# liupei101/VLSA

Measured on AMD Instinct MI355X. Metric: patches/sec per slide (50k x 512 CONCH bag), higher is better.
Workload: dtype bf16

## Files before the change

### vlsa_amd/csrc/vlfan_batch.hip

```cpp
#include "vlsa_common.h"
#ifndef VLSA_DMA_NT
#define VLSA_DMA_NT "nt"
#endif

namespace vlsa {

typedef __attribute__((address_space(3))) void* lds_void_ptr;
typedef bf16x8 __attribute__((may_alias)) bf16x8_ma;
typedef f32x4 __attribute__((may_alias)) f32x4_ma;
typedef float __attribute__((may_alias)) float_ma;
typedef int __attribute__((may_alias)) int_ma;
typedef int i32x4 __attribute__((ext_vector_type(4)));

struct BagDesc {
    const void* X;
    int64_t N;
    int64_t ldx;
};
struct RowsDesc {
    float* ptr;
    int64_t ld;
};

#ifdef VLSA_TIMING
// ... 492 lines not shown
    }
    constexpr int U = 8;
    float mx = -INFINITY;
    if (p < P)
        for (int g = 0; g < G; ++g) mx = fmaxf(mx, pm[(size_t)g * st.sm]);
    float4 a = make_float4(0.f, 0.f, 0.f, 0.f);
    float lt = 0.f;
    for (int g0 = gs; g0 < G; g0 += 2 * U) {
        float mg[U], lg[U];
        float4 v[U];
#pragma unroll
        for (int u = 0; u < U; ++u) {
            const int g = g0 + 2 * u;
            const bool ok = live && g < G;
            mg[u] = ok ? pm[(size_t)g * st.sm] : -INFINITY;
            lg[u] = ok ? pl[(size_t)g * st.sl] : 0.f;
            v[u] = ok ? *reinterpret_cast<const float4*>(pacc + (size_t)g * st.sa) : make_float4(0.f, 0.f, 0.f, 0.f);
        }
#pragma unroll
        for (int u = 0; u < U; ++u) {
            const float f = (mg[u] == -INFINITY) ? 0.f : fast_exp2(mg[u] - mx);
            lt += lg[u] * f;
            a.x += v[u].x * f; a.y += v[u].y * f; a.z += v[u].z * f; a.w += v[u].w * f;
        }
    }
    if (gs == 1) {
        sacc[p][c4] = a;
        slt[p][c4] = lt;
    }
    __syncthreads();
    if (gs == 0) {
        const float4 o = sacc[p][c4];
        a.x += o.x; a.y += o.y; a.z += o.z; a.w += o.w;
        lt += slt[p][c4];
        if (live) {
            const float inv = 1.f / lt;
            a.x *= inv; a.y *= inv; a.z *= inv; a.w *= inv;
            *reinterpret_cast<float4*>(out + (size_t)bag * st.oo + (size_t)p * D + col) = a;
            if (blockIdx.x == 0 && c4 == 0) {
                m2[(size_t)bag * st.om + p] = mx;
                l[(size_t)bag * st.ol + p] = lt;
            }
        }
    }
    if (pooled == nullptr) return;
    __syncthreads();
    if (gs == 0) sacc[p][c4] = a;
    __syncthreads();
    if (tid < 16 && col < D) {
        float4 r;
        if (pool_mode == VLSA_POOL_MAX) {
            r = sacc[0][tid];
            for (int q = 1; q < P; ++q) {
                const float4 o = sacc[q][tid];
                r.x = fmaxf(r.x, o.x); r.y = fmaxf(r.y, o.y); r.z = fmaxf(r.z, o.z); r.w = fmaxf(r.w, o.w);
            }
        } else if (pool_mode == VLSA_POOL_WEIGHT) {
            r = make_float4(0.f, 0.f, 0.f, 0.f);
            for (int q = 0; q < P; ++q) {
                const float4 o = sacc[q][tid];
                const float wq = spw[q];
                r.x += wq * o.x; r.y += wq * o.y; r.z += wq * o.z; r.w += wq * o.w;
            }
        } else {
            r = make_float4(0.f, 0.f, 0.f, 0.f);
            for (int q = 0; q < P; ++q) {
                const float4 o = sacc[q][tid];
                r.x += o.x; r.y += o.y; r.z += o.z; r.w += o.w;
            }
            const float fp = (float)P;
            r.x /= fp; r.y /= fp; r.z /= fp; r.w /= fp;
        }
        *reinterpret_cast<float4*>(pooled + (size_t)bag * D + col) = r;
    }
}

__global__ __launch_bounds__(256) void k_vlfan_merge_pool_small(const float* __restrict__ pm, const float* __restrict__ pl,
                                                                    const float* __restrict__ pacc, int G, int P, int D,
                                                                    float* __restrict__ m2, float* __restrict__ l,
                                                                    float* __restrict__ out, MergeStrides st, int pool_mode,
                                                                    const float* __restrict__ pool_w, float* __restrict__ pooled) {
    __shared__ float sm_[8][VLSA_MAX_P], sl_[8][VLSA_MAX_P];
    __shared__ float sinv[VLSA_MAX_P], spw[VLSA_MAX_P];
    __builtin_amdgcn_s_setprio(VLSA_TAIL_PRIO);
    const int tid = threadIdx.x, bag = blockIdx.x;
    pm += (size_t)bag * st.bm;
    pl += (size_t)bag * st.bl;
    pacc += (size_t)bag * st.ba;
    if (tid < 8 * VLSA_MAX_P) {
        const int g = tid >> 4, p = tid & 15;
        const bool ok = g < G && p < P;
        sm_[g][p] = ok ? pm[(size_t)g * st.sm + p] : -INFINITY;
        sl_[g][p] = ok ? pl[(size_t)g * st.sl + p] : 0.f;
    }
    if (pool_mode == VLSA_POOL_WEIGHT && tid == 255) {
        float mx = -INFINITY, sum = 0.f;
        for (int q = 0; q < P; ++q) mx = fmaxf(mx, pool_w[q]);
        for (int q = 0; q < P; ++q) { spw[q] = expf(pool_w[q] - mx); sum += spw[q]; }
        for (int q = 0; q < P; ++q) spw[q] /= sum;
    }
    __syncthreads();
    if (tid < VLSA_MAX_P) {
        const int p = tid;
        float mx = -INFINITY;
#pragma unroll
        for (int g = 0; g < 8; ++g) mx = fmaxf(mx, sm_[g][p]);
        float ls = 0.f;
#pragma unroll
        for (int g = 0; g < 8; ++g) {
            const float f = sm_[g][p] == -INFINITY ? 0.f : fast_exp2(sm_[g][p] - mx);
            ls += sl_[g][p] * f;
            sm_[g][p] = f;
        }
        sinv[p] = 1.f / ls;
        if (p < P) {
            m2[(size_t)bag * st.om + p] = mx;
            l[(size_t)bag * st.ol + p] = ls;
        }
    }
    __syncthreads();
    for (int c = tid; c < D; c += 256) {
        float acc[VLSA_MAX_P];
#pragma unroll
        for (int p = 0; p < VLSA_MAX_P; ++p) acc[p] = 0.f;
        for (int g = 0; g < G; ++g) {
            float x[VLSA_MAX_P];
#pragma unroll
            for (int p = 0; p < VLSA_MAX_P; ++p) x[p] = p < P ? pacc[(size_t)g * st.sa + (size_t)p * D + c] : 0.f;
#pragma unroll
            for (int p = 0; p < VLSA_MAX_P; ++p) acc[p] += x[p] * sm_[g][p];
        }
        float r = pool_mode == VLSA_POOL_MAX ? -INFINITY : 0.f;
#pragma unroll
        for (int p = 0; p < VLSA_MAX_P; ++p)
            if (p < P) {
                const float o = acc[p] * sinv[p];
                out[(size_t)bag * st.oo + (size_t)p * D + c] = o;
                if (pool_mode == VLSA_POOL_MAX) r = fmaxf(r, o);
                else if (pool_mode == VLSA_POOL_WEIGHT) r += spw[p] * o;
                else r += o;
            }
        if (pool_mode == VLSA_POOL_MEAN) r /= (float)P;
        if (pooled != nullptr) pooled[(size_t)bag * D + c] = r;
    }
}

__global__ __launch_bounds__(256) void k_attn_normalise_batch(const BagDesc* __restrict__ bags, const RowsDesc* __restrict__ sdesc,
                                                             const RowsDesc* __restrict__ adesc, const float* __restrict__ m2,
                                                             const float* __restrict__ l, int m_stride) {
    const int bag = blockIdx.z, p = blockIdx.y;
    const int64_t n = ((int64_t)blockIdx.x * 256 + threadIdx.x) * 4;
    const int64_t N = bags[bag].N;
    const RowsDesc sd = sdesc[bag], ad = adesc[bag];
    if (n >= N || sd.ptr == nullptr || ad.ptr == nullptr) return;
    const float m = m2[(size_t)bag * m_stride + p], inv = 1.f / l[(size_t)bag * m_stride + p];
    const f32x4 t = *reinterpret_cast<const f32x4*>(sd.ptr + (size_t)p * sd.ld + n);
    f32x4 a;
#pragma unroll
    for (int r = 0; r < 4; ++r) a[r] = fast_exp2(t[r] - m) * inv;
    *reinterpret_cast<f32x4*>(ad.ptr + (size_t)p * ad.ld + n) = a;
}

}

using namespace vlsa;

int vlsa_launch_head_batch(const float* rows, int B, int P, int D, int pool_mode, const float* pool_w, const float* W,
                           const float* b, const float* That, int K, const float* logit_scale, unsigned int* counters,
                           float* pooled, float* v, float* vhat, float* vnorm, float* logits, float* incidence,
                           hipStream_t s);
int vlsa_launch_head_pooled_batch(const float* pooled, int B, int D, const float* W, const float* b, const float* That, int K,
                                  const float* logit_scale, float* v, float* vhat, float* vnorm, float* logits,
                                  float* incidence, hipStream_t s);
int vlsa_launch_head_rows_batch(const float* rows, int B, int P, int D, int pool_mode, const float* pool_w, const float* W,
                                const float* b, const float* That, int K, const float* logit_scale, float* pooled, float* v,
                                float* vhat, float* vnorm, float* logits, float* incidence, hipStream_t s);

static int launch_merge_pool(const float* pm, const float* pl, const float* pacc, int B, int G, int P, int D, float* m2, float* l,
                             float* out, const MergeStrides& st, int pool_mode, const float* pool_w, float* pooled, hipStream_t s) {
    if (G <= 8)
        hipLaunchKernelGGL(k_vlfan_merge_pool_small, dim3(B), dim3(256), 0, s, pm, pl, pacc, G, P, D, m2, l, out, st, pool_mode, pool_w,
                           pooled);
    else
        hipLaunchKernelGGL(k_vlfan_merge_pool_batch, dim3((D + 63) / 64, B), dim3(512), 0, s, pm, pl, pacc, G, P, D, m2, l, out, st,
                           pool_mode, pool_w, pooled);
    return hipGetLastError() == hipSuccess ? VLSA_OK : VLSA_ELAUNCH;
}

#ifdef VLSA_TIMING
extern "C" int vlsa_debug_read_batch_cycles(long long* host_out) {
    return hipMemcpyFromSymbol(host_out, HIP_SYMBOL(vlsa::vlsa_dbg_batch), sizeof(long long) * 64) == hipSuccess ? 0 : -3;
}
#endif

static inline int batch_groups(int B) { return B >= 8 ? 8 : (B >= 4 ? 4 : (B >= 2 ? 2 : 1)); }
static inline int min_groups(int B) {
    int m = 1;
    while (m * bt::kMaxLocal < B) m *= 2;
    return m;
}
static inline int resolve_groups(int B, int groups) {
    int S = groups > 0 ? groups : batch_groups(B);
    int p2 = 1;
    while (p2 * 2 <= S && p2 * 2 <= B && p2 * 2 <= 256) p2 *= 2;
    const int m = min_groups(B);
    return p2 < m ? m : p2;
}
static inline int batch_workgroups(int S, int reserved_cus) {
    int r = reserved_cus < 0 ? 0 : reserved_cus;
    r = (r + S - 1) / S * S;
    if (r > 256 - S) r = 256 - S;
    return 256 - r;
}
extern "C" int vlsa_batch_partials_per_bag(int B) { return 256 / batch_groups(B); }
extern "C" int vlsa_batch_partials_per_bag_ex(int B, int reserved_cus, int groups) {
    const int S = resolve_groups(B, groups);
    return batch_workgroups(S, reserved_cus) / S;
}
extern "C" int vlsa_batch_groups(const int64_t* rows_host, int B, int reserved_cus) {
    if (!rows_host || B < 1) return 1;
    int best = 1;
    double best_cost = 1e300;
    for (int S = min_groups(B); S <= 256 && S <= B; S *= 2) {
        const int Gb = batch_workgroups(S, reserved_cus) / S;
        double worst = 0.0;
        for (int g = 0; g < S; ++g) {
            double c = 0.0;
            for (int t = g; t < B; t += S) {
                const int64_t units = (rows_host[t] + 63) / 64;
                c += (double)((units + Gb - 1) / Gb) + 0.7;
            }
            if (c > worst) worst = c;
        }
        if (worst < best_cost * 0.999) {
            best_cost = worst;
            best = S;
        }
    }
    return best;
}

extern "C" int vlsa_batch_max_bags(void) { return 64; }
extern "C" int vlsa_batch_forward_max_bags(void) { return bt::kMaxBags; }

extern "C" size_t vlsa_batch_workspace_bytes(int B, int P, int D) {
    const size_t recs = (size_t)(B < bt::kMaxLocal ? B : bt::kMaxLocal) * 256;
    return (recs * kPStride * 2 + recs * P * D) * sizeof(float) + (size_t)B * 64;
}

int vlsa_launch_partial_f32_batch(const void* bag_desc, int B, const float* qeff, const float* qmeta, int P, float* pm,
                                  float* pl, float* pacc, int S, int workgroups, const void* scores_desc, hipStream_t s);

extern "C" int vlsa_vlfan_partial_batch_scores(const void* bag_desc, int B, int x_dtype, int D, const void* qprep, int P,
                                               void* workspace, int reserved_cus, int groups, const void* scores_desc,
                                               void* stream) {
    if (!bag_desc || !qprep || !workspace) return VLSA_EINVAL;
    if (B < 1 || B > bt::kMaxBags || P < 1 || P > VLSA_MAX_P) return VLSA_EINVAL;
    if (x_dtype != VLSA_DT_BF16 && x_dtype != VLSA_DT_F32) return VLSA_EINVAL;
    if (D != 512) return VLSA_EUNSUPPORTED;
    const int S = resolve_groups(B, groups);
    const int WG = batch_workgroups(S, reserved_cus);
    const int G = WG / S;
    float* pm = static_cast<float*>(workspace);
    float* pl = pm + (size_t)B * G * kPStride;
// ... 135 lines not shown
```

### vlsa_amd/csrc/vlfan_tail.hip

```cpp
#include "vlsa_common.h"

namespace vlsa {

__global__ __launch_bounds__(256) void k_vlfan_merge(const float* __restrict__ pm, const float* __restrict__ pl,
                                                      const float* __restrict__ pacc, int G, int P, int D,
                                                      int normalise, float* __restrict__ m2, float* __restrict__ l,
                                                      float* __restrict__ out, int64_t sm, int64_t sl_, int64_t sa) {
    __shared__ float red[4];
    __shared__ __attribute__((aligned(16))) float4 sacc[16][16];
    __shared__ float sl[16];
    const int tid = threadIdx.x, lane = tid & 63, wv = tid >> 6;
    const int p = blockIdx.y, c0 = blockIdx.x * 64;
    const int c4 = tid & 15, gs = tid >> 4;
    const int col = c0 + c4 * 4;
    const bool incol = col < D;

    constexpr int U = 16;
    float mx = -INFINITY;
    float4 a = make_float4(0.f, 0.f, 0.f, 0.f);
    float lt = 0.f;
    for (int gI = tid; gI < G; gI += 256) mx = fmaxf(mx, pm[(size_t)gI * sm + p]);
    mx = wave_max(mx);
    if (lane == 0) red[wv] = mx;
    __syncthreads();
// ... 304 lines not shown
    }
    if (wv != 0) return;
    const float bj0 = bias != nullptr ? bias[j0 + i16] : 0.f, bj1 = bias != nullptr ? bias[j0 + 16 + i16] : 0.f;
#pragma unroll
    for (int r = 0; r < 4; ++r) {
        const int bg = bag0 + 4 * g + r;
        if (bg < B) {
            v[(size_t)bg * D + j0 + i16] = c0[r] + bj0;
            v[(size_t)bg * D + j0 + 16 + i16] = c1[r] + bj1;
        }
    }
}

__global__ __launch_bounds__(256) void k_head_finish(const float* __restrict__ v, int D, const float* __restrict__ That, int K,
                                                      const float* __restrict__ logit_scale, float* __restrict__ vhat,
                                                      float* __restrict__ vnorm, float* __restrict__ logits,
                                                      float* __restrict__ incidence) {
    __shared__ float sp[VLSA_MAX_D];
    __shared__ float slog[VLSA_MAX_K];
    __shared__ float red[4];
    __builtin_amdgcn_s_setprio(VLSA_TAIL_PRIO);
    const int tid = threadIdx.x, lane = tid & 63, wv = tid >> 6, bag = blockIdx.x;
    v += (size_t)bag * D;
    vhat += (size_t)bag * D;
    logits += (size_t)bag * K;
    constexpr int kTR = 4, kTC = 8;
    const bool pre = D <= 64 * kTC && K <= 4 * kTR;
    float tr[kTR][kTC];
#pragma unroll
    for (int i = 0; i < kTR; ++i)
#pragma unroll
        for (int q = 0; q < kTC; ++q) {
            const int k = wv + 4 * i, c = lane + 64 * q;
            tr[i][q] = (pre && k < K && c < D) ? That[(size_t)k * D + c] : 0.f;
        }
    const float ls_raw = logit_scale[0];
    float ss = 0.f;
    for (int c = tid; c < D; c += 256) {
        const float x = v[c];
        sp[c] = x;
        ss += x * x;
    }
    ss = block_sum_256(ss, red);
    const float nrm = fmaxf(sqrtf(ss), kNormEps);
    for (int c = tid; c < D; c += 256) {
        const float u = sp[c] / nrm;
        sp[c] = u;
        vhat[c] = u;
    }
    if (tid == 0) vnorm[bag] = nrm;
    __syncthreads();
    const float ls = expf(ls_raw);
    for (int k = wv; k < K; k += 4) {
        const float* tk = That + (size_t)k * D;
        float s = 0.f;
        if (pre) {
            const int i = (k - wv) >> 2;
#pragma unroll
            for (int ii = 0; ii < kTR; ++ii)
                if (ii == i) {
#pragma unroll
                    for (int q = 0; q < kTC; ++q)
                        if (lane + 64 * q < D) s += sp[lane + 64 * q] * tr[ii][q];
                }
        } else {
            for (int c = lane; c < D; c += 64) s += sp[c] * tk[c];
        }
        s = wave_sum(s);
        if (lane == 0) {
            const float lg = ls * s;
            logits[k] = lg;
            slog[k] = lg;
        }
    }
    __syncthreads();
    if (incidence != nullptr && tid == 0) {
        float mx = -INFINITY, s = 0.f;
        for (int k = 0; k < K; ++k) mx = fmaxf(mx, slog[k]);
        for (int k = 0; k < K; ++k) s += expf(slog[k] - mx);
        for (int k = 0; k < K; ++k) incidence[(size_t)bag * K + k] = expf(slog[k] - mx) / s;
    }
}

__global__ __launch_bounds__(256) void k_vlfan_merge_wpart(const float* __restrict__ pm, const float* __restrict__ pl,
                                                            const float* __restrict__ pacc, int G, int P, float* __restrict__ m2,
                                                            float* __restrict__ l, float* __restrict__ out,
                                                            const float* __restrict__ W, float* __restrict__ vpart) {
    constexpr int D = 512;
    constexpr unsigned sm = kPStride, sl_ = kPStride;
    const unsigned sa = (unsigned)P * D;
    const int jq = blockIdx.z;
    __shared__ float red[4];
    __shared__ __attribute__((aligned(16))) float4 sacc[16][16];
    __shared__ float sl[16];
    __builtin_amdgcn_s_setprio(VLSA_TAIL_PRIO);
    const int tid = threadIdx.x, lane = tid & 63, wv = tid >> 6;
    const int p = blockIdx.y, c0 = blockIdx.x * 64;
    const int c4 = tid & 15, gs = tid >> 4;
    const int col = c0 + c4 * 4;

    float4 wr[8];
    const float* wbase = W + (unsigned)((jq * 128 + gs * 8) * D + col);
#pragma unroll
    for (int r = 0; r < 8; ++r) wr[r] = *reinterpret_cast<const float4*>(wbase + r * D);

    constexpr int U = 16;
    float mx = -INFINITY;
    float4 a = make_float4(0.f, 0.f, 0.f, 0.f);
    float lt = 0.f;
    for (int gI = tid; gI < G; gI += 256) mx = fmaxf(mx, pm[(unsigned)gI * sm + p]);
    mx = wave_max(mx);
    if (lane == 0) red[wv] = mx;
    __syncthreads();
    mx = fmaxf(fmaxf(red[0], red[1]), fmaxf(red[2], red[3]));
    for (int g0 = gs; g0 < G; g0 += 16 * U) {
        float mg[U], lg[U];
        float4 v[U];
#pragma unroll
        for (int u = 0; u < U; ++u) {
            const unsigned gI = (unsigned)min(g0 + 16 * u, G - 1);
            mg[u] = pm[gI * sm + p];
            lg[u] = pl[gI * sl_ + p];
            v[u] = *reinterpret_cast<const float4*>(pacc + gI * sa + (unsigned)(p * D + col));
            if (g0 + 16 * u >= G) mg[u] = -INFINITY;
        }
#pragma unroll
        for (int u = 0; u < U; ++u) {
            const float f = (mg[u] == -INFINITY) ? 0.f : fast_exp2(mg[u] - mx);
            lt += lg[u] * f;
            a.x += v[u].x * f; a.y += v[u].y * f; a.z += v[u].z * f; a.w += v[u].w * f;
        }
    }
    sacc[gs][c4] = a;
    if (c4 == 0) sl[gs] = lt;
    __syncthreads();
    if (tid < 16) {
        float4 s = make_float4(0.f, 0.f, 0.f, 0.f);
        float ls = 0.f;
#pragma unroll
        for (int k = 0; k < 16; ++k) {
            const float4 v = sacc[k][tid];
            s.x += v.x; s.y += v.y; s.z += v.z; s.w += v.w;
            ls += sl[k];
        }
        const float inv = 1.f / ls;
        s.x *= inv; s.y *= inv; s.z *= inv; s.w *= inv;
        if (jq == 0) {
            *reinterpret_cast<float4*>(out + (unsigned)(p * D + c0 + tid * 4)) = s;
            if (tid == 0 && blockIdx.x == 0) {
                m2[p] = mx;
                l[p] = ls;
            }
        }
        sacc[0][tid] = s;
    }
    __syncthreads();
    const float4 o = sacc[0][c4];
    float d[8];
#pragma unroll
    for (int r = 0; r < 8; ++r) d[r] = wr[r].x * o.x + wr[r].y * o.y + wr[r].z * o.z + wr[r].w * o.w;
#pragma unroll
    for (int h = 8, n = 8; h >= 2; h >>= 1, n >>= 1) {
        const bool up = (c4 & h) != 0;
#pragma unroll
        for (int i = 0; i < n / 2; ++i) {
            const float keep = up ? d[i + n / 2] : d[i];
            const float send = up ? d[i] : d[i + n / 2];
            d[i] = keep + __shfl_xor(send, h);
        }
    }
    const float tot = d[0] + __shfl_xor(d[0], 1);
    if ((c4 & 1) == 0) vpart[(unsigned)((blockIdx.x * P + p) * D + jq * 128 + gs * 8 + (c4 >> 1))] = tot;
}

__global__ __launch_bounds__(512) void k_head_finish_parts(const float* __restrict__ vpart, const float* __restrict__ rows, int P,
                                                            int ncc, int pool_mode, const float* __restrict__ pool_w,
                                                            const float* __restrict__ bias, const float* __restrict__ That, int K,
                                                            const float* __restrict__ logit_scale, float* __restrict__ pooled,
                                                            float* __restrict__ v, float* __restrict__ vhat,
                                                            float* __restrict__ vnorm, float* __restrict__ logits,
                                                            float* __restrict__ incidence) {
    constexpr int D = 512;
    __shared__ float sp[D];
    __shared__ float swg[VLSA_MAX_P];
    __shared__ float slog[VLSA_MAX_K];
    __shared__ float red[8];
    __builtin_amdgcn_s_setprio(VLSA_TAIL_PRIO);
    const int tid = threadIdx.x, lane = tid & 63, wv = tid >> 6;
    float part[VLSA_MAX_P], x[VLSA_MAX_P];
#pragma unroll
    for (int p = 0; p < VLSA_MAX_P; ++p) {
        const unsigned pc = (unsigned)min(p, P - 1);
        float q[8];
#pragma unroll
        for (int cc = 0; cc < 8; ++cc) q[cc] = vpart[((unsigned)cc * P + pc) * D + tid];
        part[p] = ((q[0] + q[1]) + (q[2] + q[3])) + ((q[4] + q[5]) + (q[6] + q[7]));
        x[p] = rows[pc * D + tid];
    }
    const float bj = bias != nullptr ? bias[tid] : 0.f;
    if (tid == 0) {
        if (pool_mode == VLSA_POOL_WEIGHT) {
            float mx = -INFINITY, s = 0.f;
            for (int p = 0; p < P; ++p) mx = fmaxf(mx, pool_w[p]);
            for (int p = 0; p < P; ++p) { swg[p] = expf(pool_w[p] - mx); s += swg[p]; }
            for (int p = 0; p < P; ++p) swg[p] /= s;
        } else {
            for (int p = 0; p < P; ++p) swg[p] = 1.f;
        }
        for (int p = P; p < VLSA_MAX_P; ++p) swg[p] = 0.f;
    }
    __syncthreads();
    float vs = 0.f, ps = 0.f;
#pragma unroll
    for (int p = 0; p < VLSA_MAX_P; ++p) {
        vs += swg[p] * part[p];
        ps += swg[p] * x[p];
    }
    if (pool_mode == VLSA_POOL_MEAN) {
        vs /= (float)P;
        ps /= (float)P;
    }
    const float vj = vs + bj;
    pooled[tid] = ps;
    v[tid] = vj;
    float ss = wave_sum(vj * vj);
    if (lane == 0) red[wv] = ss;
    __syncthreads();
    ss = ((red[0] + red[1]) + (red[2] + red[3])) + ((red[4] + red[5]) + (red[6] + red[7]));
    const float nrm = fmaxf(sqrtf(ss), kNormEps);
    const float u = vj / nrm;
    sp[tid] = u;
    vhat[tid] = u;
    if (tid == 0) vnorm[0] = nrm;
    __syncthreads();
    const float ls = expf(logit_scale[0]);
    for (int k = wv; k < K; k += 8) {
        const float* tk = That + (size_t)k * D;
        float s = 0.f;
#pragma unroll
        for (int c = 0; c < D / 64; ++c) s += sp[lane + 64 * c] * tk[lane + 64 * c];
        s = wave_sum(s);
        if (lane == 0) {
            const float lg = ls * s;
            logits[k] = lg;
            slog[k] = lg;
        }
    }
    if (incidence == nullptr) return;
    __syncthreads();
    if (tid == 0) {
        float mx = -INFINITY, s = 0.f;
        for (int k = 0; k < K; ++k) mx = fmaxf(mx, slog[k]);
        for (int k = 0; k < K; ++k) s += expf(slog[k] - mx);
        for (int k = 0; k < K; ++k) incidence[k] = expf(slog[k] - mx) / s;
    }
}

__global__ void k_probe_mfma(float* out) {
    const int lane = threadIdx.x, g = lane >> 4, i = lane & 15;
    bf16x8 a, b;
#pragma unroll
    for (int e = 0; e < 8; ++e) {
        const int k = 8 * g + e;
        a[e] = (__bf16)((k == 5 * (i % 6)) ? (float)(i + 1) : 0.f);
        b[e] = (__bf16)(float)(4 * k + i);
    }
    f32x4 c = {0.f, 0.f, 0.f, 0.f};
    c = __builtin_amdgcn_mfma_f32_16x16x32_bf16(a, b, c, 0, 0, 0);
#pragma unroll
    for (int r = 0; r < 4; ++r) out[lane * 4 + r] = c[r];
}

__global__ void k_probe_tr(float* out) {
    __shared__ __attribute__((aligned(16))) unsigned short lds[16 * 32];
    const int lane = threadIdx.x, g = lane >> 4, i = lane & 15;
    for (int idx = lane; idx < 16 * 32; idx += 64) {
        const int row = idx >> 5, col = idx & 31;
        const __bf16 val = (__bf16)(float)((col < 16) ? (row * 16 + col) : 0);
        lds[idx] = __builtin_bit_cast(unsigned short, val);
    }
    __syncthreads();
    const unsigned short* src = lds + (4 * g + (i >> 2)) * 32 + (i & 3) * 4;
    const bf16x4 t = __builtin_amdgcn_ds_read_tr16_b64_v4bf16((lds_bf16x4_ptr)(src));
#pragma unroll
    for (int r = 0; r < 4; ++r) out[lane * 4 + r] = (float)t[r];
}

}

using namespace vlsa;

extern "C" int vlsa_abi_version(void) { return VLSA_ABI_VERSION; }

extern "C" const char* vlsa_error_string(int code) {
    switch (code) {
        case VLSA_OK: return "ok";
        case VLSA_EINVAL: return "invalid argument";
        case VLSA_EUNSUPPORTED: return "unsupported configuration";
        case VLSA_ELAUNCH: return "kernel launch failed";
        default: return "unknown error";
    }
}

static inline int launch_status() { return hipGetLastError() == hipSuccess ? VLSA_OK : VLSA_ELAUNCH; }

extern "C" int vlsa_vlfan_merge_strided(const float* pm, int64_t pm_stride, const float* pl, int64_t pl_stride,
                                        const float* pacc, int64_t pacc_stride, int G, int P, int D, int normalise,
                                        float* m2, float* l, float* out, void* stream) {
    if (!pm || !pl || !pacc || !m2 || !l || !out) return VLSA_EINVAL;
    if (G < 1 || P < 1 || P > VLSA_MAX_P || D <= 0 || D > VLSA_MAX_D || (D % 8) != 0) return VLSA_EINVAL;
    if (pm_stride < P || pl_stride < P || pacc_stride < (int64_t)P * D || (pacc_stride % 4) != 0 ||
        (reinterpret_cast<uintptr_t>(pacc) & 15) != 0)
        return VLSA_EINVAL;
    hipLaunchKernelGGL(k_vlfan_merge, dim3((D + 63) / 64, P), dim3(256), 0, (hipStream_t)stream, pm, pl, pacc, G, P, D,
                       normalise, m2, l, out, pm_stride, pl_stride, pacc_stride);
    return launch_status();
}

extern "C" int vlsa_vlfan_merge(const float* pm, const float* pl, const float* pacc, int G, int P, int D,
                                int normalise, float* m2, float* l, float* out, void* stream) {
    return vlsa_vlfan_merge_strided(pm, kPStride, pl, kPStride, pacc, (int64_t)P * D, G, P, D, normalise, m2, l, out, stream);
}

extern "C" int vlsa_attn_normalise(const float* scores, int P, int64_t N, const float* m2, const float* l, float* A,
                                   void* stream) {
    if (!scores || !m2 || !l || !A || P < 1 || P > VLSA_MAX_P || N < 0) return VLSA_EINVAL;
    if (N == 0) return VLSA_OK;
    int64_t nb = (N + 255) / 256;
    if (nb > 1024) nb = 1024;
    hipLaunchKernelGGL(k_attn_normalise, dim3((unsigned)nb, P), dim3(256), 0, (hipStream_t)stream, scores, P, N, m2, l, A);
    return launch_status();
}

extern "C" int vlsa_normalize_rows(const float* in, int rows, int D, float* out, float* norms, void* stream) {
    if (!in || !out || rows < 0 || D <= 0) return VLSA_EINVAL;
    if (rows == 0) return VLSA_OK;
    hipLaunchKernelGGL(k_normalize_rows, dim3(rows), dim3(256), 0, (hipStream_t)stream, in, D, out, norms);
    return launch_status();
}

constexpr size_t kHeadTicketBytes = 256;
extern "C" size_t vlsa_head_workspace_bytes(int D) { (void)D; return kHeadTicketBytes + (size_t)8 * VLSA_MAX_P * 512 * sizeof(float); }

extern "C" int vlsa_vlfan_merge_head(const float* pm, const float* pl, const float* pacc, int G, int P, int D, int pool_mode,
                                     const float* pool_w, const float* W, const float* b, const float* That, int K,
                                     const float* logit_scale, void* head_ws, float* m2, float* l, float* out, float* pooled,
                                     float* v, float* vhat, float* vnorm, float* logits, float* incidence, void* stream) {
    if (!pm || !pl || !pacc || !m2 || !l || !out || !That || !logit_scale || !head_ws || !pooled || !v || !vhat || !vnorm || !logits)
        return VLSA_EINVAL;
    if (G < 1 || P < 1 || P > VLSA_MAX_P || K < 1 || K > VLSA_MAX_K || D <= 0 || D > VLSA_MAX_D || (D % 8) != 0) return VLSA_EINVAL;
    if (pool_mode < VLSA_POOL_MEAN || pool_mode > VLSA_POOL_GIVEN) return VLSA_EINVAL;
    if (pool_mode == VLSA_POOL_WEIGHT && !pool_w) return VLSA_EINVAL;
    const bool fused = D == 512 && W != nullptr && (pool_mode == VLSA_POOL_MEAN || pool_mode == VLSA_POOL_WEIGHT) &&
                       (reinterpret_cast<uintptr_t>(pacc) & 15) == 0 && (reinterpret_cast<uintptr_t>(W) & 15) == 0;
    if (!fused) {
        const int rc = vlsa_vlfan_merge(pm, pl, pacc, G, P, D, 1, m2, l, out, stream);
        if (rc != VLSA_OK) return rc;
        return vlsa_head_forward(out, P, D, pool_mode, pool_w, W, b, That, K, logit_scale, head_ws, pooled, v, vhat, vnorm, logits,
                                 incidence, stream);
    }
    hipStream_t s = (hipStream_t)stream;
    float* vpart = reinterpret_cast<float*>(static_cast<unsigned char*>(head_ws) + kHeadTicketBytes);
    hipLaunchKernelGGL(k_vlfan_merge_wpart, dim3(8, P, 4), dim3(256), 0, s, pm, pl, pacc, G, P, m2, l, out, W, vpart);
    if (hipGetLastError() != hipSuccess) return VLSA_ELAUNCH;
    hipLaunchKernelGGL(k_head_finish_parts, dim3(1), dim3(512), 0, s, vpart, out, P, 8, pool_mode, pool_w, b, That, K, logit_scale,
                       pooled, v, vhat, vnorm, logits, incidence);
    return launch_status();
}

extern "C" int vlsa_head_forward(const float* rows, int P, int D, int pool_mode, const float* pool_w, const float* W,
                                 const float* b, const float* That, int K, const float* logit_scale, void* workspace,
                                 float* pooled, float* v, float* vhat, float* vnorm, float* logits, float* incidence,
                                 void* stream) {
    if (!rows || !That || !logit_scale || !workspace || !pooled || !v || !vhat || !vnorm || !logits) return VLSA_EINVAL;
    if (P < 1 || P > VLSA_MAX_P || K < 1 || K > VLSA_MAX_K || D <= 0 || D > VLSA_MAX_D || (D % 4) != 0) return VLSA_EINVAL;
    if (pool_mode < VLSA_POOL_MEAN || pool_mode > VLSA_POOL_GIVEN) return VLSA_EINVAL;
    if (pool_mode == VLSA_POOL_WEIGHT && !pool_w) return VLSA_EINVAL;
    hipStream_t s = (hipStream_t)stream;
    const int NB = W ? (D + kHeadRowsPerBlock - 1) / kHeadRowsPerBlock : 1;
    hipLaunchKernelGGL(k_head, dim3(NB), dim3(256), 0, s, rows, P, D, pool_mode, pool_w, W, b, That, K, logit_scale,
                       static_cast<unsigned int*>(workspace), pooled, v, vhat, vnorm, logits, incidence, NB);
    return launch_status();
}

int vlsa_launch_head_batch(const float* rows, int B, int P, int D, int pool_mode, const float* pool_w, const float* W,
                           const float* b, const float* That, int K, const float* logit_scale, unsigned int* counters,
                           float* pooled, float* v, float* vhat, float* vnorm, float* logits, float* incidence,
                           hipStream_t s) {
    if (pool_mode < VLSA_POOL_MEAN || pool_mode > VLSA_POOL_GIVEN) return VLSA_EINVAL;
    if (pool_mode == VLSA_POOL_WEIGHT && !pool_w) return VLSA_EINVAL;
    const int NB = W ? (D + kHeadRowsPerBlock - 1) / kHeadRowsPerBlock : 1;
    hipLaunchKernelGGL(k_head, dim3(NB, B), dim3(256), 0, s, rows, P, D, pool_mode, pool_w, W, b, That, K, logit_scale,
                       counters, pooled, v, vhat, vnorm, logits, incidence, NB);
    return launch_status();
}

int vlsa_launch_head_pooled_batch(const float* pooled, int B, int D, const float* W, const float* b, const float* That, int K,
                                  const float* logit_scale, float* v, float* vhat, float* vnorm, float* logits,
                                  float* incidence, hipStream_t s) {
    const float* vin = pooled;
    if (W != nullptr) {
        if (D == 512 && B >= 16 && (reinterpret_cast<uintptr_t>(pooled) & 15) == 0 && (reinterpret_cast<uintptr_t>(W) & 15) == 0)
            hipLaunchKernelGGL(k_head_linear_mfma, dim3((B + 15) / 16, 16), dim3(512), 0, s, pooled, B, W, b, v);
        else
            hipLaunchKernelGGL(k_head_linear, dim3((D + kHeadRowsPerBlock - 1) / kHeadRowsPerBlock, (B + kHeadBagsPerBlock - 1) / kHeadBagsPerBlock),
                               dim3(256), 0, s, pooled, B, D, W, b, v);
        vin = v;
    } else {
        if (hipMemcpyAsync(v, pooled, (size_t)B * D * sizeof(float), hipMemcpyDeviceToDevice, s) != hipSuccess) return VLSA_ELAUNCH;
    }
    hipLaunchKernelGGL(k_head_finish, dim3(B), dim3(256), 0, s, vin, D, That, K, logit_scale, vhat, vnorm, logits, incidence);
    return launch_status();
}

namespace vlsa {
__global__ __launch_bounds__(256) void k_pool_rows(const float* __restrict__ rows, int P, int D, int pool_mode,
                                                    const float* __restrict__ pool_w, float* __restrict__ pooled, int B,
                                                    const float* __restrict__ T, float* __restrict__ That, float* __restrict__ tnorm) {
    __shared__ float spw[VLSA_MAX_P];
    __shared__ float red[4];
    __builtin_amdgcn_s_setprio(VLSA_TAIL_PRIO);
    const int tid = threadIdx.x, bag = blockIdx.x;
    if (bag >= B) {
        const int r = bag - B;
        const float* x = T + (size_t)r * D;
        float ss = 0.f;
        for (int d = tid; d < D; d += 256) ss += x[d] * x[d];
        ss = block_sum_256(ss, red);
        const float nrm = fmaxf(sqrtf(ss), kNormEps);
        for (int d = tid; d < D; d += 256) That[(size_t)r * D + d] = x[d] / nrm;
        if (tnorm != nullptr && tid == 0) tnorm[r] = nrm;
        return;
    }
    if (pool_mode == VLSA_POOL_WEIGHT) {
        if (tid == 0) {
            float mx = -INFINITY, s = 0.f;
            for (int p = 0; p < P; ++p) mx = fmaxf(mx, pool_w[p]);
            for (int p = 0; p < P; ++p) { spw[p] = expf(pool_w[p] - mx); s += spw[p]; }
            for (int p = 0; p < P; ++p) spw[p] /= s;
        }
        __syncthreads();
    }
    for (int c = tid; c < D; c += 256) pooled[(size_t)bag * D + c] = pooled_col(rows + (size_t)bag * P * D, P, D, c, pool_mode, spw);
}
}
int vlsa_launch_head_rows_batch(const float* rows, int B, int P, int D, int pool_mode, const float* pool_w, const float* W,
                                const float* b, const float* That, int K, const float* logit_scale, float* pooled, float* v,
                                float* vhat, float* vnorm, float* logits, float* incidence, hipStream_t s) {
    if (pool_mode < VLSA_POOL_MEAN || pool_mode > VLSA_POOL_WEIGHT) return VLSA_EINVAL;
// ... 323 lines not shown
```

Baseline: 5.938 billion.

## Split merge-pool across column blocks and restructure fused merge-head tail kernels

The small-G merge/pool kernel now launches one block per 64-column slice per bag, not one block per bag, and stages per-prompt outputs in shared memory for pooling. The fused single-slide path replaces the merge+W-partial kernel and single-block finisher. It now uses a column-parallel fold kernel that stages exp weights in LDS, plus a 64-block head tail that computes pooled, W rows and text-dot partials, with a last-block ticket reduction. This spreads tail work across more CUs to cut serial single-block latency. The cost is more launches or blocks and atomic ticket coordination that relies on the ticket counter being preserved across calls.

```diff
diff --git a/vlsa_amd/csrc/vlfan_batch.hip b/vlsa_amd/csrc/vlfan_batch.hip
--- a/vlsa_amd/csrc/vlfan_batch.hip
+++ b/vlsa_amd/csrc/vlfan_batch.hip
@@ -598,16 +598,24 @@
                                                                     const float* __restrict__ pool_w, float* __restrict__ pooled) {
     __shared__ float sm_[8][VLSA_MAX_P], sl_[8][VLSA_MAX_P];
     __shared__ float sinv[VLSA_MAX_P], spw[VLSA_MAX_P];
+    __shared__ float so[VLSA_MAX_P][64];
     __builtin_amdgcn_s_setprio(VLSA_TAIL_PRIO);
-    const int tid = threadIdx.x, bag = blockIdx.x;
+    const int tid = threadIdx.x, bag = blockIdx.y;
+    const int p = tid >> 4, c0 = blockIdx.x * 64 + (tid & 15) * 4;
     pm += (size_t)bag * st.bm;
     pl += (size_t)bag * st.bl;
     pacc += (size_t)bag * st.ba;
+    float x[8][4];
+#pragma unroll
+    for (int g = 0; g < 8; ++g)
+#pragma unroll
+        for (int k = 0; k < 4; ++k)
+            x[g][k] = (g < G && p < P && c0 + k < D) ? pacc[(size_t)g * st.sa + (size_t)p * D + c0 + k] : 0.f;
     if (tid < 8 * VLSA_MAX_P) {
-        const int g = tid >> 4, p = tid & 15;
-        const bool ok = g < G && p < P;
-        sm_[g][p] = ok ? pm[(size_t)g * st.sm + p] : -INFINITY;
-        sl_[g][p] = ok ? pl[(size_t)g * st.sl + p] : 0.f;
+        const int g = tid >> 4, q = tid & 15;
+        const bool ok = g < G && q < P;
+        sm_[g][q] = ok ? pm[(size_t)g * st.sm + q] : -INFINITY;
+        sl_[g][q] = ok ? pl[(size_t)g * st.sl + q] : 0.f;
     }
     if (pool_mode == VLSA_POOL_WEIGHT && tid == 255) {
         float mx = -INFINITY, sum = 0.f;
@@ -617,47 +625,48 @@
     }
     __syncthreads();
     if (tid < VLSA_MAX_P) {
-        const int p = tid;
+        const int q = tid;
         float mx = -INFINITY;
 #pragma unroll
-        for (int g = 0; g < 8; ++g) mx = fmaxf(mx, sm_[g][p]);
+        for (int g = 0; g < 8; ++g) mx = fmaxf(mx, sm_[g][q]);
         float ls = 0.f;
 #pragma unroll
         for (int g = 0; g < 8; ++g) {
-            const float f = sm_[g][p] == -INFINITY ? 0.f : fast_exp2(sm_[g][p] - mx);
-            ls += sl_[g][p] * f;
-            sm_[g][p] = f;
-        }
-        sinv[p] = 1.f / ls;
-        if (p < P) {
-            m2[(size_t)bag * st.om + p] = mx;
-            l[(size_t)bag * st.ol + p] = ls;
+            const float f = sm_[g][q] == -INFINITY ? 0.f : fast_exp2(sm_[g][q] - mx);
+            ls += sl_[g][q] * f;
+            sm_[g][q] = f;
+        }
+        sinv[q] = 1.f / ls;
+        if (q < P && blockIdx.x == 0) {
+            m2[(size_t)bag * st.om + q] = mx;
+            l[(size_t)bag * st.ol + q] = ls;
         }
     }
     __syncthreads();
-    for (int c = tid; c < D; c += 256) {
-        float acc[VLSA_MAX_P];
-#pragma unroll
-        for (int p = 0; p < VLSA_MAX_P; ++p) acc[p] = 0.f;
-        for (int g = 0; g < G; ++g) {
-            float x[VLSA_MAX_P];
-#pragma unroll
-            for (int p = 0; p < VLSA_MAX_P; ++p) x[p] = p < P ? pacc[(size_t)g * st.sa + (size_t)p * D + c] : 0.f;
-#pragma unroll
-            for (int p = 0; p < VLSA_MAX_P; ++p) acc[p] += x[p] * sm_[g][p];
-        }
+    if (p < P) {
+#pragma unroll
+        for (int k = 0; k < 4; ++k) {
+            float acc = 0.f;
+#pragma unroll
+            for (int g = 0; g < 8; ++g)
+                if (g < G) acc += x[g][k] * sm_[g][p];
+            const float o = acc * sinv[p];
+            so[p][(tid & 15) * 4 + k] = o;
+            if (c0 + k < D) out[(size_t)bag * st.oo + (size_t)p * D + c0 + k] = o;
+        }
+    }
+    __syncthreads();
+    const int c = blockIdx.x * 64 + tid;
+    if (tid < 64 && c < D && pooled != nullptr) {
         float r = pool_mode == VLSA_POOL_MAX ? -INFINITY : 0.f;
-#pragma unroll
-        for (int p = 0; p < VLSA_MAX_P; ++p)
-            if (p < P) {
-                const float o = acc[p] * sinv[p];
-                out[(size_t)bag * st.oo + (size_t)p * D + c] = o;
-                if (pool_mode == VLSA_POOL_MAX) r = fmaxf(r, o);
-                else if (pool_mode == VLSA_POOL_WEIGHT) r += spw[p] * o;
-                else r += o;
-            }
+        for (int q = 0; q < P; ++q) {
+            const float o = so[q][tid];
+            if (pool_mode == VLSA_POOL_MAX) r = fmaxf(r, o);
+            else if (pool_mode == VLSA_POOL_WEIGHT) r += spw[q] * o;
+            else r += o;
+        }
         if (pool_mode == VLSA_POOL_MEAN) r /= (float)P;
-        if (pooled != nullptr) pooled[(size_t)bag * D + c] = r;
+        pooled[(size_t)bag * D + c] = r;
     }
 }
 
@@ -695,7 +704,7 @@
 static int launch_merge_pool(const float* pm, const float* pl, const float* pacc, int B, int G, int P, int D, float* m2, float* l,
                              float* out, const MergeStrides& st, int pool_mode, const float* pool_w, float* pooled, hipStream_t s) {
     if (G <= 8)
-        hipLaunchKernelGGL(k_vlfan_merge_pool_small, dim3(B), dim3(256), 0, s, pm, pl, pacc, G, P, D, m2, l, out, st, pool_mode, pool_w,
+        hipLaunchKernelGGL(k_vlfan_merge_pool_small, dim3((D + 63) / 64, B), dim3(256), 0, s, pm, pl, pacc, G, P, D, m2, l, out, st, pool_mode, pool_w,
                            pooled);
     else
         hipLaunchKernelGGL(k_vlfan_merge_pool_batch, dim3((D + 63) / 64, B), dim3(512), 0, s, pm, pl, pacc, G, P, D, m2, l, out, st,
diff --git a/vlsa_amd/csrc/vlfan_tail.hip b/vlsa_amd/csrc/vlfan_tail.hip
--- a/vlsa_amd/csrc/vlfan_tail.hip
+++ b/vlsa_amd/csrc/vlfan_tail.hip
@@ -410,177 +410,225 @@
     }
 }
 
-__global__ __launch_bounds__(256) void k_vlfan_merge_wpart(const float* __restrict__ pm, const float* __restrict__ pl,
-                                                            const float* __restrict__ pacc, int G, int P, float* __restrict__ m2,
-                                                            float* __restrict__ l, float* __restrict__ out,
-                                                            const float* __restrict__ W, float* __restrict__ vpart) {
-    constexpr int D = 512;
-    constexpr unsigned sm = kPStride, sl_ = kPStride;
-    const unsigned sa = (unsigned)P * D;
-    const int jq = blockIdx.z;
+constexpr int kFoldCols = 32;
+constexpr int kTailRows = 8;
+constexpr int kTailBlocks = 512 / kTailRows;
+constexpr unsigned kTailTicketOffset = 192;
+
+__global__ __launch_bounds__(256) void k_vlfan_fold(const float* __restrict__ pm, const float* __restrict__ pl,
+                                                     const float* __restrict__ pacc, int G, int P, float* __restrict__ m2,
+                                                     float* __restrict__ l, float* __restrict__ out) {
+    constexpr int D = 512, U = 8;
     __shared__ float red[4];
-    __shared__ __attribute__((aligned(16))) float4 sacc[16][16];
-    __shared__ float sl[16];
+    __shared__ float sf[256];
+    __shared__ __attribute__((aligned(16))) float4 sacc[4][kFoldCols / 4];
     __builtin_amdgcn_s_setprio(VLSA_TAIL_PRIO);
     const int tid = threadIdx.x, lane = tid & 63, wv = tid >> 6;
-    const int p = blockIdx.y, c0 = blockIdx.x * 64;
-    const int c4 = tid & 15, gs = tid >> 4;
-    const int col = c0 + c4 * 4;
-
-    float4 wr[8];
-    const float* wbase = W + (unsigned)((jq * 128 + gs * 8) * D + col);
-#pragma unroll
-    for (int r = 0; r < 8; ++r) wr[r] = *reinterpret_cast<const float4*>(wbase + r * D);
-
-    constexpr int U = 16;
-    float mx = -INFINITY;
+    const int p = blockIdx.y, c4 = tid & 7, gs = tid >> 3;
+    const unsigned sa = (unsigned)P * D, col = (unsigned)(p * D + blockIdx.x * kFoldCols + c4 * 4);
+    float4 v[U];
+    auto load_acc = [&](int g0) {
+#pragma unroll
+        for (int u = 0; u < U; ++u) {
+            const unsigned gI = (unsigned)min(g0 + gs + 32 * u, G - 1);
+            v[u] = *reinterpret_cast<const float4*>(pacc + gI * sa + col);
+        }
+    };
+    float mo = tid < G ? pm[(unsigned)tid * kPStride + p] : -INFINITY;
+    float lo = tid < G ? pl[(unsigned)tid * kPStride + p] : 0.f;
+    load_acc(0);
+    float mx = mo;
+    for (int gI = tid + 256; gI < G; gI += 256) mx = fmaxf(mx, pm[(unsigned)gI * kPStride + p]);
+    mx = wave_max(mx);
+    if (lane == 0) red[wv] = mx;
+    __syncthreads();
+    mx = fmaxf(fmaxf(red[0], red[1]), fmaxf(red[2], red[3]));
     float4 a = make_float4(0.f, 0.f, 0.f, 0.f);
     float lt = 0.f;
-    for (int gI = tid; gI < G; gI += 256) mx = fmaxf(mx, pm[(unsigned)gI * sm + p]);
-    mx = wave_max(mx);
-    if (lane == 0) red[wv] = mx;
-    __syncthreads();
-    mx = fmaxf(fmaxf(red[0], red[1]), fmaxf(red[2], red[3]));
-    for (int g0 = gs; g0 < G; g0 += 16 * U) {
-        float mg[U], lg[U];
-        float4 v[U];
+    for (int g0 = 0; g0 < G; g0 += 256) {
+        if (g0 > 0) {
+            __syncthreads();
+            const int gI = g0 + tid;
+            mo = gI < G ? pm[(unsigned)gI * kPStride + p] : -INFINITY;
+            lo = gI < G ? pl[(unsigned)gI * kPStride + p] : 0.f;
+            load_acc(g0);
+        }
+        const float f = mo == -INFINITY ? 0.f : fast_exp2(mo - mx);
+        lt += lo * f;
+        sf[tid] = f;
+        __syncthreads();
 #pragma unroll
         for (int u = 0; u < U; ++u) {
-            const unsigned gI = (unsigned)min(g0 + 16 * u, G - 1);
-            mg[u] = pm[gI * sm + p];
-            lg[u] = pl[gI * sl_ + p];
-            v[u] = *reinterpret_cast<const float4*>(pacc + gI * sa + (unsigned)(p * D + col));
-            if (g0 + 16 * u >= G) mg[u] = -INFINITY;
-        }
-#pragma unroll
-        for (int u = 0; u < U; ++u) {
-            const float f = (mg[u] == -INFINITY) ? 0.f : fast_exp2(mg[u] - mx);
-            lt += lg[u] * f;
-            a.x += v[u].x * f; a.y += v[u].y * f; a.z += v[u].z * f; a.w += v[u].w * f;
-        }
-    }
-    sacc[gs][c4] = a;
-    if (c4 == 0) sl[gs] = lt;
-    __syncthreads();
-    if (tid < 16) {
-        float4 s = make_float4(0.f, 0.f, 0.f, 0.f);
-        float ls = 0.f;
-#pragma unroll
-        for (int k = 0; k < 16; ++k) {
-            const float4 v = sacc[k][tid];
-            s.x += v.x; s.y += v.y; s.z += v.z; s.w += v.w;
-            ls += sl[k];
-        }
+            const float fr = sf[gs + 32 * u];
+            a.x += v[u].x * fr; a.y += v[u].y * fr; a.z += v[u].z * fr; a.w += v[u].w * fr;
+        }
+    }
+#pragma unroll
+    for (int o = 8; o < 64; o <<= 1) {
+        a.x += __shfl_xor(a.x, o); a.y += __shfl_xor(a.y, o); a.z += __shfl_xor(a.z, o); a.w += __shfl_xor(a.w, o);
+    }
+    lt = wave_sum(lt);
+    __syncthreads();
+    if (lane < kFoldCols / 4) sacc[wv][lane] = a;
+    if (lane == 0) red[wv] = lt;
+    __syncthreads();
+    if (tid < kFoldCols / 4) {
+        float4 s = sacc[0][tid];
+#pragma unroll
+        for (int k = 1; k < 4; ++k) {
+            const float4 t = sacc[k][tid];
+            s.x += t.x; s.y += t.y; s.z += t.z; s.w += t.w;
+        }
+        const float ls = (red[0] + red[1]) + (red[2] + red[3]);
         const float inv = 1.f / ls;
         s.x *= inv; s.y *= inv; s.z *= inv; s.w *= inv;
-        if (jq == 0) {
-            *reinterpret_cast<float4*>(out + (unsigned)(p * D + c0 + tid * 4)) = s;
-            if (tid == 0 && blockIdx.x == 0) {
-                m2[p] = mx;
-                l[p] = ls;
-            }
-        }
-        sacc[0][tid] = s;
-    }
-    __syncthreads();
-    const float4 o = sacc[0][c4];
-    float d[8];
-#pragma unroll
-    for (int r = 0; r < 8; ++r) d[r] = wr[r].x * o.x + wr[r].y * o.y + wr[r].z * o.z + wr[r].w * o.w;
-#pragma unroll
-    for (int h = 8, n = 8; h >= 2; h >>= 1, n >>= 1) {
-        const bool up = (c4 & h) != 0;
-#pragma unroll
-        for (int i = 0; i < n / 2; ++i) {
-            const float keep = up ? d[i + n / 2] : d[i];
-            const float send = up ? d[i] : d[i + n / 2];
-            d[i] = keep + __shfl_xor(send, h);
-        }
-    }
-    const float tot = d[0] + __shfl_xor(d[0], 1);
-    if ((c4 & 1) == 0) vpart[(unsigned)((blockIdx.x * P + p) * D + jq * 128 + gs * 8 + (c4 >> 1))] = tot;
-}
-
-__global__ __launch_bounds__(512) void k_head_finish_parts(const float* __restrict__ vpart, const float* __restrict__ rows, int P,
-                                                            int ncc, int pool_mode, const float* __restrict__ pool_w,
-                                                            const float* __restrict__ bias, const float* __restrict__ That, int K,
-                                                            const float* __restrict__ logit_scale, float* __restrict__ pooled,
-                                                            float* __restrict__ v, float* __restrict__ vhat,
-                                                            float* __restrict__ vnorm, float* __restrict__ logits,
-                                                            float* __restrict__ incidence) {
-    constexpr int D = 512;
-    __shared__ float sp[D];
-    __shared__ float swg[VLSA_MAX_P];
-    __shared__ float slog[VLSA_MAX_K];
-    __shared__ float red[8];
+        *reinterpret_cast<float4*>(out + col) = s;
+        if (tid == 0 && blockIdx.x == 0) {
+            m2[p] = mx;
+            l[p] = ls;
+        }
+    }
+}
+
+__global__ __launch_bounds__(256) void k_head_tail(const float* __restrict__ rows, int P, int pool_mode, const float* __restrict__ pool_w,
+                                                    const float* __restrict__ W, const float* __restrict__ bias,
+                                                    const float* __restrict__ That, int K, const float* __restrict__ logit_scale,
+                                                    unsigned int* ticket, float* part, float* __restrict__ pooled, float* v,
+                                                    float* __restrict__ vhat, float* __restrict__ vnorm, float* __restrict__ logits,
+                                                    float* __restrict__ incidence) {
+    constexpr int D = 512, NB = kTailBlocks, HP = VLSA_MAX_P / 2, QW = (VLSA_MAX_K + 4) / 4;
+    __shared__ __attribute__((aligned(16))) float sp[D];
+    __shared__ __attribute__((aligned(16))) float sh[D];
+    __shared__ float sv[kTailRows];
+    __shared__ float sq[VLSA_MAX_K + 1];
+    __shared__ int s_last;
     __builtin_amdgcn_s_setprio(VLSA_TAIL_PRIO);
-    const int tid = threadIdx.x, lane = tid & 63, wv = tid >> 6;
-    float part[VLSA_MAX_P], x[VLSA_MAX_P];
-#pragma unroll
-    for (int p = 0; p < VLSA_MAX_P; ++p) {
-        const unsigned pc = (unsigned)min(p, P - 1);
-        float q[8];
-#pragma unroll
-        for (int cc = 0; cc < 8; ++cc) q[cc] = vpart[((unsigned)cc * P + pc) * D + tid];
-        part[p] = ((q[0] + q[1]) + (q[2] + q[3])) + ((q[4] + q[5]) + (q[6] + q[7]));
-        x[p] = rows[pc * D + tid];
-    }
-    const float bj = bias != nullptr ? bias[tid] : 0.f;
+    const int tid = threadIdx.x, lane = tid & 63, wv = tid >> 6, jb = blockIdx.x, j0 = jb * kTailRows;
+
+    float4 wq[2][2];
+    float bj[2];
+#pragma unroll
+    for (int rr = 0; rr < 2; ++rr) {
+        const unsigned j = (unsigned)(j0 + 2 * wv + rr);
+#pragma unroll
+        for (int i = 0; i < 2; ++i) wq[rr][i] = *reinterpret_cast<const float4*>(W + j * D + lane * 4 + 256 * i);
+        bj[rr] = bias != nullptr ? bias[j] : 0.f;
+    }
+    const int c4 = tid & 127, h = tid >> 7;
+    float4 x[HP];
+#pragma unroll
+    for (int i = 0; i < HP; ++i) x[i] = *reinterpret_cast<const float4*>(rows + (unsigned)min(h + 2 * i, P - 1) * D + c4 * 4);
+    float4 t0 = make_float4(0.f, 0.f, 0.f, 0.f), t1 = t0;
+    if (tid < K) {
+        t0 = *reinterpret_cast<const float4*>(That + (unsigned)tid * D + j0);
+        t1 = *reinterpret_cast<const float4*>(That + (unsigned)tid * D + j0 + 4);
+    }
+    float wg[HP];
+    if (pool_mode == VLSA_POOL_WEIGHT) {
+        float pw[VLSA_MAX_P];
+#pragma unroll
+        for (int p = 0; p < VLSA_MAX_P; ++p) pw[p] = p < P ? pool_w[p] : -INFINITY;
+        float mx = -INFINITY, s = 0.f;
+#pragma unroll
+        for (int p = 0; p < VLSA_MAX_P; ++p) mx = fmaxf(mx, pw[p]);
+#pragma unroll
+        for (int p = 0; p < VLSA_MAX_P; ++p) s += p < P ? expf(pw[p] - mx) : 0.f;
+#pragma unroll
+        for (int i = 0; i < HP; ++i) {
+            const float e = h ? pw[2 * i + 1] : pw[2 * i];
+            wg[i] = h + 2 * i < P ? expf(e - mx) / s : 0.f;
+        }
+    } else {
+#pragma unroll
+        for (int i = 0; i < HP; ++i) wg[i] = h + 2 * i < P ? 1.f : 0.f;
+    }
+    float4 ps = make_float4(0.f, 0.f, 0.f, 0.f);
+#pragma unroll
+    for (int i = 0; i < HP; ++i) {
+        ps.x += wg[i] * x[i].x; ps.y += wg[i] * x[i].y; ps.z += wg[i] * x[i].z; ps.w += wg[i] * x[i].w;
+    }
+    if (h) *reinterpret_cast<float4*>(sh + c4 * 4) = ps;
+    __syncthreads();
+    if (!h) {
+        const float4 o = *reinterpret_cast<const float4*>(sh + c4 * 4);
+        ps.x += o.x; ps.y += o.y; ps.z += o.z; ps.w += o.w;
+        if (pool_mode == VLSA_POOL_MEAN) {
+            const float r = (float)P;
+            ps.x /= r; ps.y /= r; ps.z /= r; ps.w /= r;
+        }
+        *reinterpret_cast<float4*>(sp + c4 * 4) = ps;
+    }
+    __syncthreads();
+    if (tid < kTailRows) pooled[j0 + tid] = sp[j0 + tid];
+
+#pragma unroll
+    for (int rr = 0; rr < 2; ++rr) {
+        float s = 0.f;
+#pragma unroll
+        for (int i = 0; i < 2; ++i) {
+            const float4 q = *reinterpret_cast<const float4*>(sp + lane * 4 + 256 * i);
+            s += wq[rr][i].x * q.x + wq[rr][i].y * q.y + wq[rr][i].z * q.z + wq[rr][i].w * q.w;
+        }
+        s = wave_sum(s);
+        if (lane == 0) sv[2 * wv + rr] = s + bj[rr];
+    }
+    __syncthreads();
+    if (tid <= K) {
+        float d = 0.f;
+        if (tid < K) {
+            d = ((sv[0] * t0.x + sv[1] * t0.y) + (sv[2] * t0.z + sv[3] * t0.w)) +
+                ((sv[4] * t1.x + sv[5] * t1.y) + (sv[6] * t1.z + sv[7] * t1.w));
+        } else {
+#pragma unroll
+            for (int r = 0; r < kTailRows; ++r) d += sv[r] * sv[r];
+        }
+        __hip_atomic_store(part + (unsigned)tid * NB + jb, d, __ATOMIC_RELAXED, __HIP_MEMORY_SCOPE_AGENT);
+    } else if (tid >= 128 && tid < 128 + kTailRows) {
+        __hip_atomic_store(v + j0 + (tid - 128), sv[tid - 128], __ATOMIC_RELAXED, __HIP_MEMORY_SCOPE_AGENT);
+    }
+    asm volatile("s_waitcnt vmcnt(0)" ::: "memory");
+    __syncthreads();
     if (tid == 0) {
-        if (pool_mode == VLSA_POOL_WEIGHT) {
-            float mx = -INFINITY, s = 0.f;
-            for (int p = 0; p < P; ++p) mx = fmaxf(mx, pool_w[p]);
-            for (int p = 0; p < P; ++p) { swg[p] = expf(pool_w[p] - mx); s += swg[p]; }
-            for (int p = 0; p < P; ++p) swg[p] /= s;
-        } else {
-            for (int p = 0; p < P; ++p) swg[p] = 1.f;
-        }
-        for (int p = P; p < VLSA_MAX_P; ++p) swg[p] = 0.f;
-    }
-    __syncthreads();
-    float vs = 0.f, ps = 0.f;
-#pragma unroll
-    for (int p = 0; p < VLSA_MAX_P; ++p) {
-        vs += swg[p] * part[p];
-        ps += swg[p] * x[p];
-    }
-    if (pool_mode == VLSA_POOL_MEAN) {
-        vs /= (float)P;
-        ps /= (float)P;
-    }
-    const float vj = vs + bj;
-    pooled[tid] = ps;
-    v[tid] = vj;
-    float ss = wave_sum(vj * vj);
-    if (lane == 0) red[wv] = ss;
-    __syncthreads();
-    ss = ((red[0] + red[1]) + (red[2] + red[3])) + ((red[4] + red[5]) + (red[6] + red[7]));
-    const float nrm = fmaxf(sqrtf(ss), kNormEps);
-    const float u = vj / nrm;
-    sp[tid] = u;
-    vhat[tid] = u;
+        const unsigned int t = __hip_atomic_fetch_add(ticket, 1u, __ATOMIC_RELAXED, __HIP_MEMORY_SCOPE_AGENT);
+        s_last = ((t + 1u) % (unsigned)NB) == 0u;
+    }
+    __syncthreads();
+    if (!s_last) return;
+
+    float vv[2];
+#pragma unroll
+    for (int i = 0; i < 2; ++i) vv[i] = __hip_atomic_load(v + tid + 256 * i, __ATOMIC_RELAXED, __HIP_MEMORY_SCOPE_AGENT);
+    float q[QW];
+#pragma unroll
+    for (int i = 0; i < QW; ++i) {
+        const int qi = wv + 4 * i;
+        q[i] = qi <= K ? __hip_atomic_load(part + (unsigned)qi * NB + lane, __ATOMIC_RELAXED, __HIP_MEMORY_SCOPE_AGENT) : 0.f;
+    }
+    const float lsc = expf(logit_scale[0]);
+#pragma unroll
+    for (int i = 0; i < QW; ++i) {
+        const int qi = wv + 4 * i;
+        if (qi > K) break;
+        const float s = wave_sum(q[i]);
+        if (lane == 0) sq[qi] = s;
+    }
+    __syncthreads();
+    const float nrm = fmaxf(sqrtf(sq[K]), kNormEps);
+#pragma unroll
+    for (int i = 0; i < 2; ++i) vhat[tid + 256 * i] = vv[i] / nrm;
     if (tid == 0) vnorm[0] = nrm;
-    __syncthreads();
-    const float ls = expf(logit_scale[0]);
-    for (int k = wv; k < K; k += 8) {
-        const float* tk = That + (size_t)k * D;
-        float s = 0.f;
-#pragma unroll
-        for (int c = 0; c < D / 64; ++c) s += sp[lane + 64 * c] * tk[lane + 64 * c];
-        s = wave_sum(s);
-        if (lane == 0) {
-            const float lg = ls * s;
-            logits[k] = lg;
-            slog[k] = lg;
-        }
+    if (tid < K) {
+        const float lg = lsc * (sq[tid] / nrm);
+        logits[tid] = lg;
+        sh[tid] = lg;
     }
     if (incidence == nullptr) return;
     __syncthreads();
     if (tid == 0) {
         float mx = -INFINITY, s = 0.f;
-        for (int k = 0; k < K; ++k) mx = fmaxf(mx, slog[k]);
-        for (int k = 0; k < K; ++k) s += expf(slog[k] - mx);
-        for (int k = 0; k < K; ++k) incidence[k] = expf(slog[k] - mx) / s;
+        for (int k = 0; k < K; ++k) mx = fmaxf(mx, sh[k]);
+        for (int k = 0; k < K; ++k) s += expf(sh[k] - mx);
+        for (int k = 0; k < K; ++k) incidence[k] = expf(sh[k] - mx) / s;
     }
 }
 
@@ -680,7 +728,8 @@
     if (pool_mode < VLSA_POOL_MEAN || pool_mode > VLSA_POOL_GIVEN) return VLSA_EINVAL;
     if (pool_mode == VLSA_POOL_WEIGHT && !pool_w) return VLSA_EINVAL;
     const bool fused = D == 512 && W != nullptr && (pool_mode == VLSA_POOL_MEAN || pool_mode == VLSA_POOL_WEIGHT) &&
-                       (reinterpret_cast<uintptr_t>(pacc) & 15) == 0 && (reinterpret_cast<uintptr_t>(W) & 15) == 0;
+                       ((reinterpret_cast<uintptr_t>(pacc) | reinterpret_cast<uintptr_t>(W) | reinterpret_cast<uintptr_t>(That) |
+                         reinterpret_cast<uintptr_t>(out)) & 15) == 0;
     if (!fused) {
         const int rc = vlsa_vlfan_merge(pm, pl, pacc, G, P, D, 1, m2, l, out, stream);
         if (rc != VLSA_OK) return rc;
@@ -688,11 +737,12 @@
                                  incidence, stream);
     }
     hipStream_t s = (hipStream_t)stream;
-    float* vpart = reinterpret_cast<float*>(static_cast<unsigned char*>(head_ws) + kHeadTicketBytes);
-    hipLaunchKernelGGL(k_vlfan_merge_wpart, dim3(8, P, 4), dim3(256), 0, s, pm, pl, pacc, G, P, m2, l, out, W, vpart);
+    unsigned char* ws = static_cast<unsigned char*>(head_ws);
+    hipLaunchKernelGGL(k_vlfan_fold, dim3(512 / kFoldCols, P), dim3(256), 0, s, pm, pl, pacc, G, P, m2, l, out);
     if (hipGetLastError() != hipSuccess) return VLSA_ELAUNCH;
-    hipLaunchKernelGGL(k_head_finish_parts, dim3(1), dim3(512), 0, s, vpart, out, P, 8, pool_mode, pool_w, b, That, K, logit_scale,
-                       pooled, v, vhat, vnorm, logits, incidence);
+    hipLaunchKernelGGL(k_head_tail, dim3(kTailBlocks), dim3(256), 0, s, out, P, pool_mode, pool_w, W, b, That, K, logit_scale,
+                       reinterpret_cast<unsigned int*>(ws + kTailTicketOffset), reinterpret_cast<float*>(ws + kHeadTicketBytes), pooled, v,
+                       vhat, vnorm, logits, incidence);
     return launch_status();
 }
 
```

Result: no change. 5.935 billion (median of 6 runs) (-0.1%).
